# prismformore/Multi-Task-Transformer

Measured on AMD Instinct MI355X. Metric: training images/sec (512x512, 6 tasks), higher is better.
Workload: dtype f32(bf16x3)

## Files before the change

include/mtt_hip.h:

```cpp
#ifndef MTT_HIP_H
#define MTT_HIP_H

#include <stddef.h>
#include <stdint.h>

#ifdef __cplusplus
extern "C" {
#endif

#define MTT_ABI_VERSION 17

enum { MTT_F32 = 0, MTT_BF16 = 1, MTT_SPLIT = 2 };
enum { MTT_PREC_BF16 = 0, MTT_PREC_X3 = 1 };
enum { MTT_E_BADARG = -1, MTT_E_ALIGN = -2, MTT_E_UNSUPPORTED = -3 };

enum {
  MTT_OP_K = 0,
  MTT_OP_R = 1,
  MTT_OP_CONV_K = 2,
  MTT_OP_CONV_R = 3
};
enum { MTT_ACT_NONE = 0, MTT_ACT_GELU = 1, MTT_ACT_RELU = 2, MTT_ACT_GELU_BWD = 3, MTT_ACT_RELU_BWD = 4,
       MTT_ACT_GELU_DAUX = 5 ,
       MTT_ACT_MUL_AUX = 6    };
// ... 20 lines not shown
  int32_t M, N, K;
  int32_t a_op, b_op;
  int32_t a_dtype, b_dtype, d_dtype;
  int32_t prec;
  int64_t lda, ldb, ldd;
  int32_t a_mb; int64_t a_bs;
  int32_t d_mb; int64_t d_bs;
  int32_t batch, batch_inner;
  int64_t a_zo, a_zi, b_zo, b_zi, d_zo, d_zi;
  mtt_conv_geom conv;
  float alpha;
  const float* colscale; const float* colshift; int64_t col_zo, col_zi;
  int32_t act;
  const void* aux_in; void* aux_out; int32_t aux_dtype; int64_t ldaux; int64_t aux_zo, aux_zi;
  const float* rowscale; int32_t n_prompt;
  const float* resid; int64_t ldr; int32_t r_mb; int64_t r_bs; int64_t r_zo, r_zi;
  int32_t n_store;
  int32_t store_mode;
  int32_t ps_H, ps_W, ps_Co;
  int32_t variant;
  const void* A_lo; const void* B_lo; void* D_lo;
  float* colsum_out; float* colsum_ws;
  const float* a_scale; const float* a_shift; int32_t a_act; void* a_aux16; int64_t ld_a16;
} mtt_gemm_desc;
size_t mtt_gemm_colsum_ws_floats(const mtt_gemm_desc* d);

int mtt_abi_version(void);
size_t mtt_desc_size(int which);
int mtt_gemm(const mtt_gemm_desc* d, void* stream);
int mtt_gemm_variant(const mtt_gemm_desc* d);

typedef struct {
  const void* qkv; void* out; float* rawlog; float* lse;
  int32_t B, N, nH, T;
  int32_t dtype, prec;
  float scale;
  int32_t variant;
  const void* qkv_lo; void* out_lo;
} mtt_attn_desc;
int mtt_attn_fwd(const mtt_attn_desc* d, void* stream);
int mtt_attn_bwd(const mtt_attn_desc* d, const void* dout, const float* drawlog, void* dqkv, float* stat, void* stream);

typedef struct {
  const void* S; void* P; const void* dP; void* dS; const float* extra;
  int64_t rows, cols, ld; int32_t s_dtype, p_dtype; float scale;
  int64_t rows_per_mat; int32_t extra_rows; int64_t extra_ld;
} mtt_softmax_desc;
int mtt_softmax_fwd(const mtt_softmax_desc* d, void* stream);
int mtt_softmax_bwd(const mtt_softmax_desc* d, void* stream);

typedef struct {
  const float* x; void* y; const float* gamma; const float* beta; float* mean; float* rstd;
  const void* dy; float* dx; float* dgamma; float* dbeta;
// ... 317 lines not shown
```

multi-task-transformer_amd/_lib.py:

```python
import ctypes as C
import os

import torch

_HERE = os.path.dirname(os.path.abspath(__file__))
LIB_PATH = os.path.join(_HERE, "libmtt_hip.so")

ABI_VERSION = 17
F32, BF16, SPLIT = 0, 1, 2
PREC_BF16, PREC_X3 = 0, 1
OP_K, OP_R, OP_CONV_K, OP_CONV_R = 0, 1, 2, 3
ACT_NONE, ACT_GELU, ACT_RELU, ACT_GELU_BWD, ACT_RELU_BWD, ACT_GELU_DAUX, ACT_MUL_AUX = 0, 1, 2, 3, 4, 5, 6
STORE_ROWS, STORE_PIXSHUF2 = 0, 1
GEMM_AUTO, GEMM_GENERAL, GEMM_DMA256, GEMM_DMA128, GEMM_GENERAL_EPILOGUE = 0, 1, 3, 4, 11
ATTN_AUTO, ATTN_PLAIN = 0, 1

i32, i64, f32, ptr = C.c_int32, C.c_int64, C.c_float, C.c_void_p


class ConvGeom(C.Structure):
    _fields_ = [("H", i32), ("W", i32), ("C", i32), ("Cp", i32), ("dil", i32), ("flip", i32)]


class GemmDesc(C.Structure):
# ... 1 lines not shown
        ("A", ptr), ("B", ptr), ("D", ptr),
        ("M", i32), ("N", i32), ("K", i32),
        ("a_op", i32), ("b_op", i32),
        ("a_dtype", i32), ("b_dtype", i32), ("d_dtype", i32),
        ("prec", i32),
        ("lda", i64), ("ldb", i64), ("ldd", i64),
        ("a_mb", i32), ("a_bs", i64),
        ("d_mb", i32), ("d_bs", i64),
        ("batch", i32), ("batch_inner", i32),
        ("a_zo", i64), ("a_zi", i64), ("b_zo", i64), ("b_zi", i64), ("d_zo", i64), ("d_zi", i64),
        ("conv", ConvGeom),
        ("alpha", f32),
        ("colscale", ptr), ("colshift", ptr), ("col_zo", i64), ("col_zi", i64),
        ("act", i32),
        ("aux_in", ptr), ("aux_out", ptr), ("aux_dtype", i32), ("ldaux", i64), ("aux_zo", i64), ("aux_zi", i64),
        ("rowscale", ptr), ("n_prompt", i32),
        ("resid", ptr), ("ldr", i64), ("r_mb", i32), ("r_bs", i64), ("r_zo", i64), ("r_zi", i64),
        ("n_store", i32), ("store_mode", i32),
        ("ps_H", i32), ("ps_W", i32), ("ps_Co", i32),
        ("variant", i32),
        ("A_lo", ptr), ("B_lo", ptr), ("D_lo", ptr),
        ("colsum_out", ptr), ("colsum_ws", ptr),
        ("a_scale", ptr), ("a_shift", ptr), ("a_act", i32), ("a_aux16", ptr), ("ld_a16", i64),
    ]


class AttnDesc(C.Structure):
    _fields_ = [("qkv", ptr), ("out", ptr), ("rawlog", ptr), ("lse", ptr),
                ("B", i32), ("N", i32), ("nH", i32), ("T", i32), ("dtype", i32), ("prec", i32), ("scale", f32),
                ("variant", i32), ("qkv_lo", ptr), ("out_lo", ptr)]


class SoftmaxDesc(C.Structure):
    _fields_ = [("S", ptr), ("P", ptr), ("dP", ptr), ("dS", ptr), ("extra", ptr),
                ("rows", i64), ("cols", i64), ("ld", i64), ("s_dtype", i32), ("p_dtype", i32), ("scale", f32),
                ("rows_per_mat", i64), ("extra_rows", i32), ("extra_ld", i64)]


class LnDesc(C.Structure):
    _fields_ = [("x", ptr), ("y", ptr), ("gamma", ptr), ("beta", ptr), ("mean", ptr), ("rstd", ptr),
                ("dy", ptr), ("dx", ptr), ("dgamma", ptr), ("dbeta", ptr),
                ("rows", i64), ("C", i32), ("ldx", i64), ("ldy", i64), ("y_dtype", i32), ("eps", f32), ("dx_in", ptr), ("ws", ptr),
                ("y_lo", ptr), ("y32", ptr), ("ldy32", i64)]


class ChanLogitDesc(C.Structure):
# ... 335 lines not shown
    return t.data_ptr()


def _stream():
    return torch.cuda.current_stream().cuda_stream


def gemm_variant(**kw):
    lib = load()
    desc = GemmDesc()
    for k, v in kw.items():
        if k == "conv":
            for ck, cv in v.items():
                setattr(desc.conv, ck, int(cv))
        elif isinstance(v, torch.Tensor):
            setattr(desc, k, v.data_ptr())
        elif v is not None:
            setattr(desc, k, v)
    lib.mtt_gemm_variant.restype = C.c_int
    lib.mtt_gemm_variant.argtypes = [C.POINTER(GemmDesc)]
    return lib.mtt_gemm_variant(C.byref(desc))


def call(name, **kw):
    lib = load()
    fn = getattr(lib, "mtt_" + name)
    if name in POSITIONAL:
        args = [(_addr(a) if isinstance(a, torch.Tensor) else a) for a in kw["args"]]
        rc = fn(*args, _stream())
    else:
        extra = None
        if name in DESC_EXTRA:
            st, _ = DESC_EXTRA[name]
            desc = st()
            extra = [(_addr(a) if isinstance(a, torch.Tensor) else a) for a in kw["xargs"]]
        else:
            desc = (POSTPROC[name] if name in POSTPROC else EVAL[name] if name in EVAL else DESCS[name])()
        for k, v in kw.items():
            if k == "xargs":
                continue
            if k == "in":
                k = "in_"
            if k == "conv":
                for ck, cv in v.items():
                    setattr(desc.conv, ck, int(cv))
            elif isinstance(v, torch.Tensor):
# ... 13 lines not shown
```

multi-task-transformer_amd/autograd_path.py:

```python
import math

import torch
import torch.distributed as dist
import torch.nn as nn
from torch.autograd import Function

from . import bn as bn_mod
from . import _lib, ops
from ._lib import ACT_GELU, ACT_GELU_BWD, ACT_GELU_DAUX, ACT_MUL_AUX, ACT_NONE, F32, OP_CONV_R, OP_K, OP_R, dtype_code

pitch = ops.pitch
SPLITK_MIN_ROWS = 4096
WGRAD_MAX_SLICES, WGRAD_TARGET_WGS = 192, 512


def _gemm(A, B, D, M, N, K, prec, **kw):
    args = dict(A=A, B=B, D=D, M=M, N=N, K=K, a_op=OP_K, b_op=OP_K, a_dtype=dtype_code(A), b_dtype=dtype_code(B),
                d_dtype=dtype_code(D), prec=prec.code, batch=1, batch_inner=1, alpha=1.0)
    args.update(kw)
    ops.call("gemm", **args)
    return D


def _colsum(x2d, cols):
    return ops.colsum(x2d, cols)


def _scaled(g, rowscale, mb, n_prompt, prec):
    if rowscale is None and (g.dtype == prec.adt or not FAST_BWD):
        return g
    out = torch.empty(g.shape, dtype=prec.adt, device=g.device)
    ops.call("rowscale_cast", args=[g, out, g.shape[0], g.shape[1], g.stride(0), out.stride(0), dtype_code(g), dtype_code(out),
                                    rowscale, mb, n_prompt])
    return out


def _scaled_colsum(g, rowscale, mb, n_prompt, prec):
    cols = g.shape[1]
    if (rowscale is None and (g.dtype == prec.adt or not FAST_BWD)) or cols % 8 or g.stride(0) % 8:
        out = _scaled(g, rowscale, mb, n_prompt, prec)
        return out, _colsum(out, cols)
    out = torch.empty(g.shape, dtype=prec.adt, device=g.device)
    cs = torch.empty(cols, dtype=torch.float32, device=g.device)
    ws = ops.workspace(_lib.load().mtt_rowscale_cast_colsum_ws_floats(g.shape[0], cols), g.device)
    ops.call("rowscale_cast_colsum", args=[g, out, g.shape[0], cols, g.stride(0), out.stride(0), dtype_code(g), dtype_code(out),
                                           rowscale, mb, n_prompt, cs, ws])
    return out, cs


def _to_bwd(t, prec):
    if prec.name != "bf16" or t.dtype != torch.float32 or not FAST_BWD:
        return t
    t2 = t.reshape(-1, t.shape[-1])
    return ops.cast_rows(t2, torch.bfloat16).view(t.shape)


def _wgrad(dy, x, N, Kp, prec, rows=None, lda=None, ldb=None):
    rows = rows if rows is not None else dy.shape[0]
    lda, ldb = lda or dy.stride(0), ldb or x.stride(0)
    tiles = -(-N // 128) * -(-Kp // 128)
    if tiles < 96 and rows >= SPLITK_MIN_ROWS:
        Z = max(2, min(WGRAD_MAX_SLICES, WGRAD_TARGET_WGS // tiles, max(2, rows // 512)))
        c = rows // Z
        rem = rows - c * Z
        slabs = torch.empty(Z + (1 if rem else 0), N, Kp, dtype=torch.float32, device=dy.device)
        _gemm(dy, x, slabs, N, Kp, c, prec, a_op=OP_R, b_op=OP_R, lda=lda, ldb=ldb, ldd=Kp, batch=Z, a_zo=c * lda, b_zo=c * ldb,
              d_zo=N * Kp)
        if rem:
            _gemm(dy[c * Z:], x[c * Z:], slabs[Z], N, Kp, rem, prec, a_op=OP_R, b_op=OP_R, lda=lda, ldb=ldb, ldd=Kp)
        return slabs.sum(0)
# ... 220 lines not shown
        else:
            cq = ops.linear(xn, wt, hw, ps, bias=btt[None], a_rows=(T, N * C, C), M=B * T)[0]
        if side:
            xnc = xn if split or ps.adt == xn.dtype else ops.cast2d(xn, xn.shape[0], C, C, ps.adt, ldd=C)
            rawchan = ops.chan_logits(cq, xnc, B, T, N, C, (h, w), (nwin, nwin))
        pr = XT2.view(B, N, C)[:, :T]
        ops.linear(cq, wt1, C, ps, bias=btt1[None], out=pr, d_rows=(T, N * C, C), resid=pr, rowscale=rowscale, n_prompt=T, M=B * T)
    saved = (XT, g1, mean, rstd, ops._hi(xn), ops._hi(qkv), ops._hi(ao), ops._hi(wq), ops._hi(wp), rowscale, lse, cq, wt, wt1, xp32) if keep else None
    return (XT2, rawlog, rawchan), saved


def mlp_half(XT2, g2, b2n, eps, W1, b1, W2, b2, rowscale, geo, prec, tag, *, keep, pe=None):
    B, N, T = geo
    pe = pe or prec
    assert not keep or pe.name == prec.name
    C, Hd = W1.shape[1], W1.shape[0]
    split = prec.split and ((C % 64 == 0 and Hd % 64 == 0) if MLP_SPLIT_RULE64 else (ops.split_gemm_ok(C) and ops.split_gemm_ok(Hd)))
    odt = "split" if split else prec.adt
    xn2, mean, rstd = ops.layernorm(XT2, g2, b2n, eps, prec, save_stats=keep, out_dtype=odt)
    w1 = ops.pack_linear([W1], pe, tag + ('fc1',), split=split)
    w2 = ops.pack_linear([W2], pe, tag + ('fc2',), split=split)
    z = torch.empty(B * N, Hd, dtype=prec.bwd.adt, device=XT2.device) if keep else None
    daux = keep and GELU_DAUX and z.dtype == torch.bfloat16
    hmid = ops.linear(xn2, w1, Hd, pe, bias=b1[None], act=ACT_GELU_DAUX if daux else ACT_GELU, aux_out=z, out_dtype=odt)[0]
    XT3 = torch.empty_like(XT2)
    rows = dict(d_rows=(N, N * C, C), M=B * N) if keep or rowscale is not None else {}
    ops.linear(hmid, w2, C, pe, bias=b2[None], out=XT3, resid=XT2, rowscale=rowscale, n_prompt=T, **rows)
    saved = (XT2, g2, mean, rstd, ops._hi(xn2), z, ops._hi(hmid), ops._hi(w1), ops._hi(w2), rowscale) if keep else None
    return XT3, saved


class AttnHalfFn(Function):

    @staticmethod
    def forward(ctx, XT, g1, b1, eps, Wqkv, bqkv, Wproj, bproj, Wtt, btt, Wtt1, btt1, rowscale, geo, prec, tag):
        (XT2, rawlog, rawchan), saved = attn_half(XT, g1, b1, eps, Wqkv, bqkv, Wproj, bproj, Wtt, btt, Wtt1, btt1, rowscale, geo, prec, tag, keep=True)
        ctx.save_for_backward(*saved)
        ctx.geo, ctx.prec, ctx.eps, ctx.chan = geo, prec, eps, Wtt is not None
        ctx.params = (Wqkv, Wproj, Wtt, Wtt1)
        ctx.set_materialize_grads(False)
        z = torch.zeros(0, device=XT.device)
        return XT2, (rawlog if rawlog is not None else z), (rawchan if rawchan is not None else z)

    @staticmethod
    def backward(ctx, dXT2, drawlog, drawchan):
        XT, g1, mean, rstd, xn, qkv, ao, wq, wp, rowscale, lse, cq, wt, wt1, xp32 = ctx.saved_tensors
        Wqkv_, Wproj_, Wtt_, Wtt1_ = ctx.params
        B, N, nH, T, h, w, nwin = ctx.geo[:7]
        prec, C, M, hw = ctx.prec.bwd, nH * 64, B * N, h * w
        xn_c = xn
        if dXT2 is None:
            dXT2 = torch.zeros_like(XT)
        dXT2 = dXT2.contiguous()
        g, dbproj = _scaled_colsum(dXT2, rowscale, N, T, prec)
        dWproj, _ = _enc_wgrad(g, ao, C, C, prec, bias=False)
        dao = _enc_dgrad(g, Wproj_, wp[0], M, C, C, prec, prec.adt, 'proj')
        dl = drawlog.contiguous() if (T > 0 and drawlog is not None and drawlog.numel()) else None
        if lse is not None:
            dqkv = attention_bwd_flash(qkv, ao, lse, dao, dl, B, N, nH, T, prec)
        else:
            dqkv = attention_bwd(qkv, dao, dl, B, N, nH, T, prec)
        dWqkv, dbqkv = _enc_wgrad(dqkv, xn, 3 * C, C, prec)
        dxn = _enc_dgrad(dqkv, Wqkv_, wq[0], M, C, 3 * C, prec, torch.float32, 'qkv')
        dWtt = dbtt = dWtt1 = dbtt1 = None
        if ctx.chan:
            hwp = cq.shape[-1]
            gp = dXT2.view(B, N, C)[:, :T].reshape(B * T, C)
            if rowscale is not None:
                gp = gp * rowscale[:, 0].repeat_interleave(T)[:, None]
            dWtt1 = _wgrad(gp, cq, C, hwp, prec)[:, :hw]
            dbtt1 = _colsum(gp, C)
            fast_tt = prec.name == "bf16" and FAST_BWD and hwp == hw and hw >= FAST_MIN_DIM and C >= FAST_MIN_DIM and C % 64 == 0
            if fast_tt:
                gp16 = ops.cast_rows(gp, torch.bfloat16)
                dcq = _enc_dgrad(gp16, Wtt1_, wt1[0], B * T, hwp, C, prec, torch.float32, 'tt1')
            else:
                dcq = _dgrad(gp, wt1[0], B * T, hwp, C, prec, torch.float32)
            if drawchan is not None and drawchan.numel():
                dq2 = torch.zeros(B * T, hwp, dtype=torch.float32, device=xn.device)
# ... 18 lines not shown


class MlpHalfFn(Function):

    @staticmethod
    def forward(ctx, XT2, g2, b2n, eps, W1, b1, W2, b2, rowscale, geo, prec, tag):
        XT3, saved = mlp_half(XT2, g2, b2n, eps, W1, b1, W2, b2, rowscale, geo, prec, tag, keep=True)
        ctx.save_for_backward(*saved)
        ctx.geo, ctx.prec, ctx.eps, ctx.daux = geo, prec, eps, GELU_DAUX and saved[5].dtype == torch.bfloat16
        ctx.params = (W1, W2)
        return XT3

    @staticmethod
    def backward(ctx, dXT3):
        XT2, g2, mean, rstd, xn2, z, hmid, w1, w2, rowscale = ctx.saved_tensors
        B, N, T = ctx.geo
        prec, M = ctx.prec.bwd, B * N
        C, Hd = xn2.shape[1], z.shape[1]
        dXT3 = dXT3.contiguous()
        g, db2 = _scaled_colsum(dXT3, rowscale, N, T, prec)
        W1_, W2_ = ctx.params
        dW2, _ = _enc_wgrad(g, hmid, C, Hd, prec, bias=False)
        dz, db1 = _enc_dgrad(g, W2_, w2[0], M, Hd, C, prec, prec.adt, 'fc2', colsum=True, act=ACT_MUL_AUX if ctx.daux else ACT_GELU_BWD, aux_in=z,
                             aux_dtype=dtype_code(z), ldaux=Hd)
        dW1, _ = _enc_wgrad(dz, xn2, Hd, C, prec, bias=False)
        dxn2 = _enc_dgrad(dz, W1_, w1[0], M, C, Hd, prec, prec.adt, 'fc1')
        dXT2, dg2, dbn2 = _ln_bwd_join(dXT3, XT2, dxn2, g2, mean, rstd, ctx.eps)
        return dXT2, dg2, dbn2, None, dW1, db1, dW2, db2, None, None, None, None


def block_attn(keep, gp, *args):
    return AttnHalfFn.apply(*args) if keep else attn_half(*args, keep=False, gp=gp)[0]


def block_mlp(keep, pe, *args):
    return MlpHalfFn.apply(*args) if keep else mlp_half(*args, keep=False, pe=pe)[0]


def patch_embed(img, Wpe, bpe, pos, first, geo, prec, tag, pe=None):
    B, N, T, hw = geo
    C = Wpe.shape[0]
    XT = torch.empty(B * N, C, dtype=torch.float32, device=img.device)
    XT.view(B, N, C)[:, :T] = first
    cols = ops.patchify(img.float(), prec)
    wpe = ops.pack_linear([Wpe], pe or prec, tag)
    ops.linear(cols, wpe, C, pe or prec, bias=bpe[None], out=XT.view(B, N, C)[:, T:], d_rows=(hw, N * C, C),
               resid=pos[0, 1:], r_rows=(hw, 0, C), M=B * hw)
    return XT, cols

# ... 700 lines not shown
```

multi-task-transformer_amd/csrc/gemm.hip:

```cpp
#include "mtt_device.h"
#include <type_traits>

namespace {

#ifndef MTT_GROUP_M
#define MTT_GROUP_M 4
#endif
#ifndef MTT_RING
#define MTT_RING 1
#endif
constexpr int BM = 128, BN = 128, BK = 64;
constexpr int TILE_BYTES = BM * BK * 2;

struct GemmP {
  mtt_gemm_desc d;
  FastDiv divW, divH, divCp, div3;
  FastDiv divAmb, divDmb, divRmb;
  FastDiv divPsW, divPsH, divPsCo;
  int tiles_m, tiles_n;
  int group_m;
#ifdef MTT_GEMM_TRACE
  unsigned long long* trace;
#endif
};

#ifdef MTT_GEMM_TRACE
MTT_DEV unsigned long long trace_hwid() {
  unsigned a, b;
  asm volatile("s_getreg_b32 %0, hwreg(HW_REG_HW_ID)" : "=s"(a));
  asm volatile("s_getreg_b32 %0, hwreg(HW_REG_XCC_ID)" : "=s"(b));
  return (unsigned long long)a | ((unsigned long long)b << 32);
}
#define MTT_TRACE(slot) do { if (p.trace && threadIdx.x == 0) p.trace[(size_t)(blockIdx.x + gridDim.x * blockIdx.z) * 8 + (slot)] = __builtin_amdgcn_s_memtime(); } while (0)
#define MTT_TRACE_RT(slot) do { if (p.trace && threadIdx.x == 0) p.trace[(size_t)(blockIdx.x + gridDim.x * blockIdx.z) * 8 + (slot)] = __builtin_amdgcn_s_memrealtime(); } while (0)
#define MTT_TRACE_ID(tile) do { if (p.trace && threadIdx.x == 0) { p.trace[(size_t)(blockIdx.x + gridDim.x * blockIdx.z) * 8 + 6] = trace_hwid(); p.trace[(size_t)(blockIdx.x + gridDim.x * blockIdx.z) * 8 + 7] = (tile); } } while (0)
#else
#define MTT_TRACE(slot) do {} while (0)
#define MTT_TRACE_RT(slot) do {} while (0)
#define MTT_TRACE_ID(tile) do {} while (0)
#endif

MTT_DEV int64_t row_off(uint32_t m, int mb, int64_t bs, int64_t ld, FastDiv f) {
  if (mb <= 0) return (int64_t)m * ld;
  const uint32_t q = fdiv(m, f);
  return (int64_t)q * bs + (int64_t)(m - q * (uint32_t)mb) * ld;
}


__device__ __attribute__((aligned(32))) const unsigned g_zero_page[8] = {0u, 0u, 0u, 0u, 0u, 0u, 0u, 0u};

template <bool X3, bool CONV, bool F32>
struct StagerK {
  const void* base; int dtype; int K; int c;
  int64_t roff[4]; bool rok[4];
  uint64_t zpage;
  unsigned tapmask[4];
  int tap, ci, knext;
  Raw8<F32> raw[4];

  MTT_DEV void init(const GemmP& p, const void* b, int dt, int row0, int rows, int64_t ld, int mb, int64_t bs, FastDiv fmb) {
    base = b; dtype = dt; K = p.d.K; c = threadIdx.x & 7;
    zpage = (uint64_t)(uintptr_t)g_zero_page;
    asm volatile("" : "+s"(zpage));
#pragma unroll
    for (int i = 0; i < 4; ++i) {
      const int r = row0 + (threadIdx.x >> 3) + 32 * i;
      rok[i] = r < rows;
      const uint32_t rr = rok[i] ? (uint32_t)r : 0u;
// ... 699 lines not shown
    } else {
      const int k0 = s * BK;
#pragma unroll
      for (int i = 0; i < 4; ++i) {
        const uint64_t src = (uint64_t)(uintptr_t)(Abase + (aoff[i] + k0));
        glds16((const bf16_t*)(uintptr_t)(k0 + ack[i] < K ? src : zpage), sA + i * 1024);
      }
#pragma unroll
      for (int i = 0; i < 4; ++i) {
        const uint64_t src = (uint64_t)(uintptr_t)(Bbase + (boff[i] + k0));
        glds16((const bf16_t*)(uintptr_t)(k0 + ack[i] < K ? src : zpage), sB + i * 1024);
      }
    }
  };

  f32x4 acc[MT][NT];
#pragma unroll
  for (int a = 0; a < MT; ++a)
#pragma unroll
    for (int b = 0; b < NT; ++b) acc[a][b] = (f32x4){0.f, 0.f, 0.f, 0.f};

  const int nk = X3CAT ? 3 * (K / BK) : (K + BK - 1) / BK;
  issue(0, 0);
  asm volatile("s_waitcnt vmcnt(0)" ::: "memory");
  __builtin_amdgcn_s_barrier();
  MTT_TRACE(2);
  if (late) __builtin_amdgcn_s_barrier();
  __builtin_amdgcn_sched_barrier(0);

  auto main_loop = [&](auto late_tag) {
  (void)late_tag;
  for (int kt = 0; kt < nk; ++kt) {
    const unsigned char* Ah = smem + (kt & 1) * STAGE;
    const unsigned char* Bh = Ah + TILE_A;
#pragma unroll
    for (int kh = 0; kh < 2; ++kh) {
      if (kh == 0 && kt + 1 < nk) issue((kt + 1) & 1, kt + 1);
      u32x4 fa[MT], fb[NT];
#pragma unroll
      for (int t = 0; t < NT; ++t) fb[t] = *(const u32x4*)(Bh + lds_off(wn * 64 + t * 16 + li, kh * 4 + lg));
#pragma unroll
      for (int t = 0; t < MT; ++t) fa[t] = *(const u32x4*)(Ah + lds_off(wm * (MT * 16) + t * 16 + li, kh * 4 + lg));
      if (kh == 1) asm volatile("s_waitcnt vmcnt(0) lgkmcnt(0)" ::: "memory");
      else asm volatile("s_waitcnt lgkmcnt(0)" ::: "memory");
      __builtin_amdgcn_sched_barrier(0);
      __builtin_amdgcn_s_barrier();
      __builtin_amdgcn_sched_barrier(0);
      __builtin_amdgcn_s_setprio(1);
#pragma unroll
      for (int a = 0; a < MT; ++a)
#pragma unroll
        for (int b = 0; b < NT; ++b) acc[a][b] = mfma16(fa[a], fb[b], acc[a][b]);
      __builtin_amdgcn_s_setprio(0);
      __builtin_amdgcn_sched_barrier(0);
      __builtin_amdgcn_s_barrier();
      __builtin_amdgcn_sched_barrier(0);
    }
  }
  };
  if (late) main_loop(std::true_type{}); else main_loop(std::false_type{});
  if (!late) __builtin_amdgcn_s_barrier();
  __syncthreads();
  MTT_TRACE(3);
  gemm_epilogue_auto<256, WAVES_M, WAVES_N, MT, NT>(p, acc, smem, m0, n0, zo, zi);
  MTT_TRACE(4); MTT_TRACE_RT(5); MTT_TRACE_ID(tile_m * tiles_n + tile_n);
}

template <int ADDR>
int launch_dma(const GemmP& p, hipStream_t stream) {
  constexpr int smem = (BM2 * BK * 2 + 256 * BK * 2) * 2;
  static std::atomic<unsigned long long> done{0};
  if (int e = mtt_ensure_dyn_lds((const void*)gemm_dma_kernel<ADDR>, smem, done)) return e;
  const int tm = (p.d.M + BM2 - 1) / BM2, tn = (p.d.N + 255) / 256;
  dim3 grid(tm * tn, 1, p.d.batch);
  hipLaunchKernelGGL((gemm_dma_kernel<ADDR>), grid, dim3(512), smem, stream, p);
  return (int)hipGetLastError();
}

MTT_DEV int ring_swz(int row) { return (0x78 >> (((row >> 2) & 3) * 2)) & 3; }

#define MTT_VMCNT_CASE(n) case n: asm volatile("s_waitcnt vmcnt(" #n ")" ::: "memory"); break;
MTT_DEV void wait_vmcnt_dyn(int n) {
  switch (n) {
    MTT_VMCNT_CASE(24) MTT_VMCNT_CASE(22) MTT_VMCNT_CASE(20) MTT_VMCNT_CASE(18) MTT_VMCNT_CASE(16) MTT_VMCNT_CASE(14) MTT_VMCNT_CASE(12)
// ... 70 lines not shown
#pragma unroll
      for (int i = 0; i < 2; ++i) {
        const uint64_t src = (uint64_t)(uintptr_t)(base + aoff32[i]);
        glds16((const bf16_t*)(uintptr_t)(((tapmask[i] >> tap) & 1u) ? src : zpage), dst + i * 1024);
      }
      return;
    }
    const unsigned char* base = (part == 0 ? AbaseH : part == 1 ? BbaseH : part == 2 ? BbaseL : AbaseL) + (size_t)j * 64;
    glds16((const bf16_t*)(base + (isA ? aoff32[0] : boff32[0])), dst);
    if (isA || !EDGE) glds16((const bf16_t*)(base + (isA ? aoff32[1] : boff32[1])), dst + 1024);
  };
  const int fsw = ((lg ^ ring_swz(li)) << 4) + li * 64;
  const int fragA = wm * (MT * 16) * 64 + fsw, fragB = wn * (NT * 16) * 64 + fsw;

  f32x4 acc[MT][NT];
#pragma unroll
  for (int a = 0; a < MT; ++a)
#pragma unroll
    for (int b = 0; b < NT; ++b) acc[a][b] = (f32x4){0.f, 0.f, 0.f, 0.f};

  constexpr int W_BL = 3 * NA + 2 * NB, W_AL = 3 * NA + 3 * NB, W_AB = 2 * NA + 3 * NB;
  issue_part(0, 0); issue_part(0, 1); issue_part(0, 2); issue_part(0, 3);
  issue_part(1, 0); issue_part(1, 1); issue_part(1, 2);
  wait_vmcnt_imm<2 * NA + 3 * NB>();
  __builtin_amdgcn_s_barrier();
  if (late) __builtin_amdgcn_s_barrier();
  __builtin_amdgcn_sched_barrier(0);

#define MTT_R3_CLOSE() do { __builtin_amdgcn_sched_barrier(0); __builtin_amdgcn_s_barrier(); __builtin_amdgcn_sched_barrier(0); } while (0)
  auto main_loop = [&](auto late_tag) {
  constexpr bool LATE = decltype(late_tag)::value;
  for (int j = 0; j < nk; ++j) {
    const unsigned char* sb = smem + (j & 1) * SLOT;
    const bool m1 = j + 1 < nk, m2 = j + 2 < nk;
    const int w_bl = NA + (m1 ? 2 * NA + 2 * NB : 0), w_al = (m1 ? 2 * NA + 2 * NB : 0) + (m2 ? NA + NB : 0), w_ab = NA + NB + (m2 ? NA + 2 * NB : 0);
    u32x4 fa[MT], fbh[NT], fbl[NT];
    if (m1) issue_part(j + 1, 3);
#pragma unroll
    for (int t = 0; t < NT; ++t) fbh[t] = *(const u32x4*)(sb + PART + fragB + t * 1024);
#pragma unroll
    for (int t = 0; t < MT; ++t) fa[t] = *(const u32x4*)(sb + fragA + t * 1024);
    if (LATE) { if (m2) wait_vmcnt_imm<W_BL>(); else wait_vmcnt_dyn(w_bl); }
    asm volatile("s_waitcnt lgkmcnt(0)" ::: "memory");
    MTT_R3_CLOSE();
    __builtin_amdgcn_s_setprio(1);
#pragma unroll
// ... 16 lines not shown
      for (int b = 0; b < NT; ++b) acc[a][b] = mfma16(fa[a], fbl[b], acc[a][b]);
    __builtin_amdgcn_s_setprio(0);
    if (!LATE) { if (m2) wait_vmcnt_imm<W_AL>(); else wait_vmcnt_dyn(w_al); }
    MTT_R3_CLOSE();
    if (m2) issue_part(j + 2, 2);
#pragma unroll
    for (int t = 0; t < MT; ++t) fa[t] = *(const u32x4*)(sb + 3 * PART + fragA + t * 1024);
    if (LATE) { if (m2) wait_vmcnt_imm<W_AB>(); else wait_vmcnt_dyn(w_ab); }
    asm volatile("s_waitcnt lgkmcnt(0)" ::: "memory");
    MTT_R3_CLOSE();
    __builtin_amdgcn_s_setprio(1);
#pragma unroll
    for (int a = 0; a < MT; ++a)
#pragma unroll
      for (int b = 0; b < NT; ++b) acc[a][b] = mfma16(fa[a], fbh[b], acc[a][b]);
    __builtin_amdgcn_s_setprio(0);
    if (!LATE) { if (m2) wait_vmcnt_imm<W_AB>(); else wait_vmcnt_dyn(w_ab); }
    MTT_R3_CLOSE();
  }
  };
#undef MTT_R3_CLOSE
  if (late) main_loop(std::true_type{}); else main_loop(std::false_type{});
  if (!late) __builtin_amdgcn_s_barrier();
  __syncthreads();
  if constexpr (EDGE) gemm_epilogue<128, WAVES_M, WAVES_N, MT, NT>(p, acc, smem, m0, n0, zo, zi);
  else gemm_epilogue_auto<256, WAVES_M, WAVES_N, MT, NT>(p, acc, smem, m0, n0, zo, zi);
}

template <bool CONV>
__global__ __launch_bounds__(512, 1) void gemm_ring3_kernel(const GemmP p) {
  extern __shared__ __attribute__((aligned(16))) unsigned char smem[];
  const int wg = xcd_remap(blockIdx.x, gridDim.x);
  const int tiles_n = (p.d.N + 255) / 256, tiles_m = (p.d.M + BM2 - 1) / BM2;
  int tile_m, tile_n;
  grouped_tile(wg, tiles_m, tiles_n, p.group_m, tile_m, tile_n);
  const int m0 = tile_m * BM2, n0 = tile_n * 256;
  const int z = blockIdx.z;
  const int zo = z / p.d.batch_inner, zi = z - zo * p.d.batch_inner;
  const int ncols = (p.d.n_store > p.d.N ? p.d.n_store : p.d.N) - n0;
  if (MTT_R3_EDGE && ncols <= 128 && p.d.store_mode == MTT_STORE_ROWS) ring3_tile<CONV, true>(p, smem, m0, n0, zo, zi);
  else ring3_tile<CONV, false>(p, smem, m0, n0, zo, zi);
}

template <bool CONV>
int launch_ring3(const GemmP& p, hipStream_t stream) {
  constexpr int smem = 2 * 4 * 16384;
// ... 629 lines not shown
    if (fills && 100 * (int64_t)d.M * d.N >= 45 * pm * pn) return 6;
    return 0;
  }
  const bool dma = d.a_op == MTT_OP_K && d.b_op == MTT_OP_K && (d.K % 8) == 0;
  if (!dma || d.variant == MTT_GEMM_GENERAL) return 0;
  if (d.variant == MTT_GEMM_DMA256) return 3;
  if (d.variant == MTT_GEMM_DMA128) return 4;
  const int n256 = (d.N + 255) / 256 * 256, n128 = (d.N + 127) / 128 * 128;
  const bool wide = 100 * n128 > 85 * n256;
  const int batch = d.batch < 1 ? 1 : d.batch;
  const int64_t blocks = (int64_t)((d.M + 255) / 256) * ((d.N + 255) / 256) * batch;
  if (wide && d.M >= 512 && d.N >= 512 && blocks >= 96) return 3;
  const int tbn = 32 * dma128_nt(d);
  const int64_t blocks128 = (int64_t)((d.M + 127) / 128) * ((d.N + tbn - 1) / tbn) * batch;
  if (d.M >= 512 && d.K >= 128 && blocks128 >= 256) return 4;
  if (d.M >= 128 && d.N >= 256 && d.K >= 512) return 4;
  return 0;
}
#ifdef MTT_GEMM_TRACE
static unsigned long long* g_trace_host = nullptr;
extern "C" void mtt_debug_set_trace(void* buf) { g_trace_host = (unsigned long long*)buf; }
#endif
extern "C" int mtt_gemm_variant(const mtt_gemm_desc* d) { return d ? gemm_variant_for(*d) : MTT_E_BADARG; }

static int gemm_launch(GemmP& p, hipStream_t s, int v);
extern "C" int mtt_gemm(const mtt_gemm_desc* dd, void* stream) {
  if (!dd || !dd->A || !dd->B || !dd->D) return MTT_E_BADARG;
  GemmP p; p.d = *dd;
  mtt_gemm_desc& d = p.d;
  if (d.M <= 0 || d.N <= 0 || d.K <= 0) return MTT_E_BADARG;
  if (d.batch < 1) d.batch = 1;
  if (d.batch_inner < 1) d.batch_inner = 1;
  const bool a_k = d.a_op == MTT_OP_K || d.a_op == MTT_OP_CONV_K, b_k = d.b_op == MTT_OP_K;
  const int Kp8 = (d.K + 7) / 8 * 8;
  if ((a_k && d.a_op == MTT_OP_K && d.lda < Kp8) || (b_k && d.ldb < Kp8)) return MTT_E_ALIGN;
  if (d.a_op == MTT_OP_CONV_K && (d.K % 8)) return MTT_E_ALIGN;
  if ((d.lda % 8) || (d.ldb % 8)) return MTT_E_ALIGN;
  if (((uintptr_t)d.A & 15) || ((uintptr_t)d.B & 15)) return MTT_E_ALIGN;
  if ((d.aux_in || d.aux_out) && (d.ldaux <= 0 || (d.ldaux % 8))) return MTT_E_BADARG;
  if (d.act < MTT_ACT_NONE || d.act > MTT_ACT_MUL_AUX) return MTT_E_BADARG;
  if ((d.act == MTT_ACT_GELU_DAUX && !d.aux_out) || ((d.act == MTT_ACT_MUL_AUX || d.act == MTT_ACT_GELU_BWD || d.act == MTT_ACT_RELU_BWD) && !d.aux_in))
    return MTT_E_BADARG;
  if ((d.ldd % 8) || ((uintptr_t)d.D & 15) || (d.d_bs % 8) || (d.d_zo % 8) || (d.d_zi % 8)) return MTT_E_ALIGN;
  if (d.resid && ((d.ldr % 4) || ((uintptr_t)d.resid & 15) || (d.r_bs % 4))) return MTT_E_ALIGN;
  const bool conv = d.a_op == MTT_OP_CONV_K || d.b_op == MTT_OP_CONV_R;
  if (conv) {
    if (d.conv.H <= 0 || d.conv.W <= 0 || d.conv.Cp % 8 || d.conv.C > d.conv.Cp || d.conv.dil < 1) return MTT_E_BADARG;
    if (d.a_op == MTT_OP_CONV_K && d.K != 9 * d.conv.Cp) return MTT_E_BADARG;
    if (d.b_op == MTT_OP_CONV_R && d.N != 9 * d.conv.Cp) return MTT_E_BADARG;
  }
  if (d.store_mode == MTT_STORE_PIXSHUF2 && (d.ps_H <= 0 || d.ps_W <= 0 || d.ps_Co <= 0 || d.N != 4 * d.ps_Co)) return MTT_E_BADARG;
  p.divW = make_div(conv ? d.conv.W : 1); p.divH = make_div(conv ? d.conv.H : 1);
  p.divCp = make_div(conv ? d.conv.Cp : 1); p.div3 = make_div(3);
  p.divAmb = make_div(d.a_mb > 0 ? d.a_mb : 1); p.divDmb = make_div(d.d_mb > 0 ? d.d_mb : 1);
  p.divRmb = make_div(d.r_mb > 0 ? d.r_mb : 1);
  p.divPsW = make_div(d.ps_W > 0 ? d.ps_W : 1); p.divPsH = make_div(d.ps_H > 0 ? d.ps_H : 1);
  p.divPsCo = make_div(d.ps_Co > 0 ? d.ps_Co : 1);
  p.tiles_m = (d.M + BM - 1) / BM; p.tiles_n = (d.N + BN - 1) / BN;
  p.group_m = MTT_GROUP_M;
#ifdef MTT_GEMM_TRACE
  p.trace = g_trace_host;
#endif
  hipStream_t s = (hipStream_t)stream;
  const int v = gemm_variant_for(d);
  if (v < 0) return v;
  if (d.d_dtype == MTT_SPLIT && !d.D_lo) return MTT_E_BADARG;
  if (d.d_dtype == MTT_SPLIT && d.store_mode != MTT_STORE_ROWS) return MTT_E_UNSUPPORTED;
  if (d.colsum_out) {
    if (!d.colsum_ws) return MTT_E_BADARG;
    if (d.batch != 1 || d.store_mode != MTT_STORE_ROWS || v == 6) return MTT_E_UNSUPPORTED;
    const int rc = gemm_launch(p, s, v);
    if (rc) return rc;
    const int tbm = (v == 3 || v == 8 || v == 9) ? 256 : BM;
    hipLaunchKernelGGL(mtt_colsum_final_kernel, dim3((d.N + 31) / 32, 1, 1), dim3(256), 0, s, (const float*)d.colsum_ws, d.colsum_out, d.N,
                       (d.M + tbm - 1) / tbm, (int64_t)0);
    return (int)hipGetLastError();
  }
  return gemm_launch(p, s, v);
}

// ... 46 lines not shown
```

multi-task-transformer_amd/ops.py:

```python
import weakref

import torch

from . import _lib
from ._lib import (ACT_GELU, ACT_NONE, ACT_RELU, BF16, F32, OP_CONV_K, OP_CONV_R, OP_K, OP_R, PREC_BF16, PREC_X3, SPLIT)


PITCH32_FROM = 160


def pitch(n):
    return (n + 31) // 32 * 32 if n >= PITCH32_FROM else (n + 7) // 8 * 8


DEFAULT_PREC = "x3f"


class Prec:

    def __init__(self, name):
        assert name in ("bf16", "x3", "x3f")
        self.name = name
        self.code = PREC_BF16 if name == "bf16" else PREC_X3
        self.adt = torch.bfloat16 if name == "bf16" else torch.float32
# ... 371 lines not shown
    mode, dt = _mode(prec, split)
    return seg_pack((tag, mode, 'kmap', tuple(id(w) for w in weights)), list(weights),
                    lambda: _dest((Z, N, Kp), dt, weights[0].device),
                    lambda buf: [segment(w, s0, buf, z * N * Kp + d0, (1, N, ln), (0, K, 1), (0, Kp, 1))
                                 for z, w in enumerate(weights) for (d0, s0, ln) in kmap],
                    check=lambda: _check_sources(weights, lambda w: w.numel() == N * K))


def stack_vec(vs, tag):
    n, Z = vs[0].numel(), len(vs)
    if any(v.dtype != torch.float32 or not v.is_contiguous() or v.numel() != n for v in vs):
        def build():
            with torch.no_grad():
                return torch.stack([v.detach().float().reshape(-1) for v in vs], 0).contiguous()
        return _cached((tag, tuple(id(v) for v in vs)), vs, build)
    return seg_pack((tag, 'vec', tuple(id(v) for v in vs)), list(vs),
                    lambda: torch.zeros(Z, n, dtype=torch.float32, device=vs[0].device),
                    lambda buf: [segment(v, 0, buf, z * n, (1, 1, n), (0, 0, 1), (0, 0, 1)) for z, v in enumerate(vs)])



def linear(x, wpack, N, prec, *, bias=None, act=ACT_NONE, out=None, out_dtype=None, M=None,
           a_rows=None, d_rows=None, resid=None, r_rows=None, rowscale=None, n_prompt=0, aux_out=None, aux_in=None,
           colscale=None, alpha=1.0, batch_inner=1, d_z=None, ldd=None, n_store=None, a_affine=None):
    Z, Nw, Kp = wpack.shape
    assert N <= Nw
    x_split = isinstance(x, Split)
    assert x_split == isinstance(wpack, Split), "split planes: both operands or neither"
    if a_rows is not None:
        a_mb, a_bs, lda = a_rows
        a_z = 0
    else:
        xh = _hi(x)
        xv = xh if xh.dim() == 3 else xh[None]
        if M is None:
            M = xv.shape[1]
        a_mb, a_bs, lda = 0, 0, xv.shape[2]
        a_z = xv.stride(0) if xv.shape[0] > 1 else 0
        assert xv.shape[0] in (1, Z) and lda >= Kp
    Np = ldd if (out is None and ldd is not None) else pitch(N)
    if out is None:
        out = Split.empty((Z, M, Np), x.device) if out_dtype == "split" else torch.empty(Z, M, Np, dtype=out_dtype or prec.adt, device=x.device)
    oh = _hi(out)
    if d_rows is not None:
        d_mb, d_bs, ldd_ = d_rows
        dz = 0
        nst = N
# ... 13 lines not shown
        kw.update(A_lo=x.lo, B_lo=wpack.lo)
    if isinstance(out, Split):
        kw.update(D_lo=out.lo)
    kw.update(a_zo=a_z * batch_inner, a_zi=a_z if batch_inner > 1 else 0,
              b_zo=wh.stride(0) * batch_inner, b_zi=wh.stride(0) if batch_inner > 1 else 0)
    if d_z is not None:
        kw.update(d_zo=d_z[0], d_zi=d_z[1])
    else:
        kw.update(d_zo=dz * batch_inner, d_zi=dz if batch_inner > 1 else 0)
    if bias is not None or colscale is not None:
        ref = bias if bias is not None else colscale
        cz = ref.stride(0) if (ref.dim() == 2 and ref.shape[0] > 1) else 0
        kw.update(colshift=bias, colscale=colscale, col_zo=cz * batch_inner, col_zi=cz if batch_inner > 1 else 0)
    if resid is not None:
        rr = r_rows if r_rows is not None else (d_mb, d_bs, ldd_)
        kw.update(resid=resid, r_mb=rr[0], r_bs=rr[1], ldr=rr[2])
    if rowscale is not None:
        kw.update(rowscale=rowscale, n_prompt=n_prompt)
    if aux_out is not None or aux_in is not None:
        aux = aux_out if aux_out is not None else aux_in
        az = aux.stride(0) if aux.dim() == 3 else 0
        kw.update(aux_out=aux_out, aux_in=aux_in, aux_dtype=dtype_code(aux), ldaux=aux.shape[-1],
                  aux_zo=az * batch_inner, aux_zi=az if batch_inner > 1 else 0)
    if a_affine is not None:
        sc, sh, a_act, a16 = a_affine
        kw.update(a_scale=sc, a_shift=sh, a_act=a_act, a_aux16=a16, ld_a16=a16.stride(-2) if a16 is not None else 0)
    call("gemm", **kw)
    return out


def head_prologue_ok(rows, K, n, lda):
    return GEMM_VARIANT is None and n <= 32 and K % 8 == 0 and K <= 1024 and rows >= 1 and lda % 4 == 0


SPLIT_CONV_MAX_ELEMS = 2 ** 31 - 1


def conv3x3(x, wpack, Co, Ci, B, H, W, prec, *, bias=None, colscale=None, act=ACT_NONE, dil=1, flip=0, out_dtype=None):
    Z, rows, Cp = x.shape
    assert rows == B * H * W and wpack.shape[-1] == 9 * Cp
    if isinstance(wpack, Split) and not isinstance(x, Split):
        x = x.float().contiguous()
        sp = split_cast(x.view(Z * rows, Cp))
        x = Split(sp.hi.view(Z, rows, Cp), sp.lo.view(Z, rows, Cp))
    assert isinstance(x, Split) == isinstance(wpack, Split), "split planes: both operands or neither"
    Cop = pitch(Co)
# ... 262 lines not shown
```

Before: 189.0.

## Skip GEMM main loop for row tiles fully zeroed by drop-path rowscale

Adds a per-tile check in two GEMM kernel paths that reads the per-sample rowscale table. When every row in a 128-row tile belongs to a sample whose drop-path scale is zero, the K-loop is skipped and only the epilogue runs on a zero accumulator. Encoder MLP fc1 forward and the proj, fc2 and fc1 dgrad calls pass this table as a hint, so samples dropped by stochastic depth stop costing matrix math. The cost is a small per-tile table read, plus reliance on downstream rowscale masking to zero out the bias/activation values that are still written for skipped rows. A runtime toggle is exposed for debugging.

```diff
diff --git a/include/mtt_hip.h b/include/mtt_hip.h
--- a/include/mtt_hip.h
+++ b/include/mtt_hip.h
@@ -66,6 +66,7 @@
   const void* A_lo; const void* B_lo; void* D_lo;
   float* colsum_out; float* colsum_ws;
   const float* a_scale; const float* a_shift; int32_t a_act; void* a_aux16; int64_t ld_a16;
+  const float* skip_scale; int32_t skip_mb, skip_np;
 } mtt_gemm_desc;
 size_t mtt_gemm_colsum_ws_floats(const mtt_gemm_desc* d);
 
@@ -73,6 +74,7 @@
 size_t mtt_desc_size(int which);
 int mtt_gemm(const mtt_gemm_desc* d, void* stream);
 int mtt_gemm_variant(const mtt_gemm_desc* d);
+int mtt_debug_set_gemm_rowskip(int on);
 
 typedef struct {
   const void* qkv; void* out; float* rawlog; float* lse;
diff --git a/multi-task-transformer_amd/_lib.py b/multi-task-transformer_amd/_lib.py
--- a/multi-task-transformer_amd/_lib.py
+++ b/multi-task-transformer_amd/_lib.py
@@ -47,6 +47,7 @@
         ("A_lo", ptr), ("B_lo", ptr), ("D_lo", ptr),
         ("colsum_out", ptr), ("colsum_ws", ptr),
         ("a_scale", ptr), ("a_shift", ptr), ("a_act", i32), ("a_aux16", ptr), ("ld_a16", i64),
+        ("skip_scale", ptr), ("skip_mb", i32), ("skip_np", i32),
     ]
 
 
@@ -428,6 +429,13 @@
     return lib.mtt_gemm_variant(C.byref(desc))
 
 
+def set_gemm_rowskip(on):
+    lib = load()
+    lib.mtt_debug_set_gemm_rowskip.restype = C.c_int
+    lib.mtt_debug_set_gemm_rowskip.argtypes = [C.c_int]
+    return bool(lib.mtt_debug_set_gemm_rowskip(1 if on else 0))
+
+
 def call(name, **kw):
     lib = load()
     fn = getattr(lib, "mtt_" + name)
diff --git a/multi-task-transformer_amd/autograd_path.py b/multi-task-transformer_amd/autograd_path.py
--- a/multi-task-transformer_amd/autograd_path.py
+++ b/multi-task-transformer_amd/autograd_path.py
@@ -46,6 +46,12 @@
     ops.call("rowscale_cast_colsum", args=[g, out, g.shape[0], cols, g.stride(0), out.stride(0), dtype_code(g), dtype_code(out),
                                            rowscale, mb, n_prompt, cs, ws])
     return out, cs
+
+
+def _skip_hint(rowscale, mb, n_prompt):
+    if rowscale is None or not rowscale.is_cuda:
+        return {}
+    return dict(skip_scale=rowscale, skip_mb=mb, skip_np=n_prompt)
 
 
 def _to_bwd(t, prec):
@@ -312,7 +318,8 @@
     w2 = ops.pack_linear([W2], pe, tag + ('fc2',), split=split)
     z = torch.empty(B * N, Hd, dtype=prec.bwd.adt, device=XT2.device) if keep else None
     daux = keep and GELU_DAUX and z.dtype == torch.bfloat16
-    hmid = ops.linear(xn2, w1, Hd, pe, bias=b1[None], act=ACT_GELU_DAUX if daux else ACT_GELU, aux_out=z, out_dtype=odt)[0]
+    hmid = ops.linear(xn2, w1, Hd, pe, bias=b1[None], act=ACT_GELU_DAUX if daux else ACT_GELU, aux_out=z, out_dtype=odt,
+                      row_skip=_skip_hint(rowscale, N, T))[0]
     XT3 = torch.empty_like(XT2)
     rows = dict(d_rows=(N, N * C, C), M=B * N) if keep or rowscale is not None else {}
     ops.linear(hmid, w2, C, pe, bias=b2[None], out=XT3, resid=XT2, rowscale=rowscale, n_prompt=T, **rows)
@@ -344,7 +351,7 @@
         dXT2 = dXT2.contiguous()
         g, dbproj = _scaled_colsum(dXT2, rowscale, N, T, prec)
         dWproj, _ = _enc_wgrad(g, ao, C, C, prec, bias=False)
-        dao = _enc_dgrad(g, Wproj_, wp[0], M, C, C, prec, prec.adt, 'proj')
+        dao = _enc_dgrad(g, Wproj_, wp[0], M, C, C, prec, prec.adt, 'proj', **_skip_hint(rowscale, N, T))
         dl = drawlog.contiguous() if (T > 0 and drawlog is not None and drawlog.numel()) else None
         if lse is not None:
             dqkv = attention_bwd_flash(qkv, ao, lse, dao, dl, B, N, nH, T, prec)
@@ -409,9 +416,9 @@
         W1_, W2_ = ctx.params
         dW2, _ = _enc_wgrad(g, hmid, C, Hd, prec, bias=False)
         dz, db1 = _enc_dgrad(g, W2_, w2[0], M, Hd, C, prec, prec.adt, 'fc2', colsum=True, act=ACT_MUL_AUX if ctx.daux else ACT_GELU_BWD, aux_in=z,
-                             aux_dtype=dtype_code(z), ldaux=Hd)
+                             aux_dtype=dtype_code(z), ldaux=Hd, **_skip_hint(rowscale, N, T))
         dW1, _ = _enc_wgrad(dz, xn2, Hd, C, prec, bias=False)
-        dxn2 = _enc_dgrad(dz, W1_, w1[0], M, C, Hd, prec, prec.adt, 'fc1')
+        dxn2 = _enc_dgrad(dz, W1_, w1[0], M, C, Hd, prec, prec.adt, 'fc1', **_skip_hint(rowscale, N, T))
         dXT2, dg2, dbn2 = _ln_bwd_join(dXT3, XT2, dxn2, g2, mean, rstd, ctx.eps)
         return dXT2, dg2, dbn2, None, dW1, db1, dW2, db2, None, None, None, None
 
diff --git a/multi-task-transformer_amd/csrc/gemm.hip b/multi-task-transformer_amd/csrc/gemm.hip
--- a/multi-task-transformer_amd/csrc/gemm.hip
+++ b/multi-task-transformer_amd/csrc/gemm.hip
@@ -9,6 +9,9 @@
 #ifndef MTT_RING
 #define MTT_RING 1
 #endif
+#ifndef MTT_GEMM_ROWSKIP
+#define MTT_GEMM_ROWSKIP 1
+#endif
 constexpr int BM = 128, BN = 128, BK = 64;
 constexpr int TILE_BYTES = BM * BK * 2;
 
@@ -17,6 +20,9 @@
   FastDiv divW, divH, divCp, div3;
   FastDiv divAmb, divDmb, divRmb;
   FastDiv divPsW, divPsH, divPsCo;
+  const float* skip_tab;
+  int skip_mb, skip_np;
+  FastDiv divSkip;
   int tiles_m, tiles_n;
   int group_m;
 #ifdef MTT_GEMM_TRACE
@@ -44,6 +50,20 @@
   if (mb <= 0) return (int64_t)m * ld;
   const uint32_t q = fdiv(m, f);
   return (int64_t)q * bs + (int64_t)(m - q * (uint32_t)mb) * ld;
+}
+
+MTT_DEV bool rows_all_dropped(const GemmP& p, int m0, int m1) {
+  if (!MTT_GEMM_ROWSKIP || !p.skip_tab) return false;
+  uint32_t q = fdiv((uint32_t)m0, p.divSkip);
+  int r0 = m0 - (int)q * p.skip_mb;
+  for (int m = m0; m < m1; ++q) {
+    const int left = m1 - m, room = p.skip_mb - r0;
+    const int n = left < room ? left : room;
+    if (r0 < p.skip_np && p.skip_tab[2 * q] != 0.0f) return false;
+    if (r0 + n > p.skip_np && p.skip_tab[2 * q + 1] != 0.0f) return false;
+    m += n; r0 = 0;
+  }
+  return true;
 }
 
 
@@ -789,8 +809,10 @@
 
   const int nk = X3CAT ? 3 * (K / BK) : (K + BK - 1) / BK;
   issue(0, 0);
+  const bool dropped = ADDR == 1 && rows_all_dropped(p, m0, m0 + BM2 < p.d.M ? m0 + BM2 : p.d.M);
   asm volatile("s_waitcnt vmcnt(0)" ::: "memory");
   __builtin_amdgcn_s_barrier();
+  if (!dropped) {
   MTT_TRACE(2);
   if (late) __builtin_amdgcn_s_barrier();
   __builtin_amdgcn_sched_barrier(0);
@@ -827,6 +849,7 @@
   };
   if (late) main_loop(std::true_type{}); else main_loop(std::false_type{});
   if (!late) __builtin_amdgcn_s_barrier();
+  }
   __syncthreads();
   MTT_TRACE(3);
   gemm_epilogue_auto<256, WAVES_M, WAVES_N, MT, NT>(p, acc, smem, m0, n0, zo, zi);
@@ -943,6 +966,9 @@
   constexpr int W_BL = 3 * NA + 2 * NB, W_AL = 3 * NA + 3 * NB, W_AB = 2 * NA + 3 * NB;
   issue_part(0, 0); issue_part(0, 1); issue_part(0, 2); issue_part(0, 3);
   issue_part(1, 0); issue_part(1, 1); issue_part(1, 2);
+  const bool dropped = !CONV && rows_all_dropped(p, m0, m0 + BM2 < p.d.M ? m0 + BM2 : p.d.M);
+  if (dropped) asm volatile("s_waitcnt vmcnt(0)" ::: "memory");
+  else {
   wait_vmcnt_imm<2 * NA + 3 * NB>();
   __builtin_amdgcn_s_barrier();
   if (late) __builtin_amdgcn_s_barrier();
@@ -1005,6 +1031,7 @@
 #undef MTT_R3_CLOSE
   if (late) main_loop(std::true_type{}); else main_loop(std::false_type{});
   if (!late) __builtin_amdgcn_s_barrier();
+  }
   __syncthreads();
   if constexpr (EDGE) gemm_epilogue<128, WAVES_M, WAVES_N, MT, NT>(p, acc, smem, m0, n0, zo, zi);
   else gemm_epilogue_auto<256, WAVES_M, WAVES_N, MT, NT>(p, acc, smem, m0, n0, zo, zi);
@@ -1680,6 +1707,8 @@
 extern "C" void mtt_debug_set_trace(void* buf) { g_trace_host = (unsigned long long*)buf; }
 #endif
 extern "C" int mtt_gemm_variant(const mtt_gemm_desc* d) { return d ? gemm_variant_for(*d) : MTT_E_BADARG; }
+static std::atomic<int> g_rowskip_on{1};
+extern "C" int mtt_debug_set_gemm_rowskip(int on) { return g_rowskip_on.exchange(on ? 1 : 0); }
 
 static int gemm_launch(GemmP& p, hipStream_t s, int v);
 extern "C" int mtt_gemm(const mtt_gemm_desc* dd, void* stream) {
@@ -1714,6 +1743,13 @@
   p.divRmb = make_div(d.r_mb > 0 ? d.r_mb : 1);
   p.divPsW = make_div(d.ps_W > 0 ? d.ps_W : 1); p.divPsH = make_div(d.ps_H > 0 ? d.ps_H : 1);
   p.divPsCo = make_div(d.ps_Co > 0 ? d.ps_Co : 1);
+  if (d.skip_scale && (d.skip_mb <= 0 || d.skip_np < 0)) return MTT_E_BADARG;
+  p.skip_tab = nullptr; p.skip_mb = 1; p.skip_np = 0;
+  if (g_rowskip_on.load(std::memory_order_relaxed)) {
+    if (d.rowscale && d.d_mb > 0) { p.skip_tab = d.rowscale; p.skip_mb = d.d_mb; p.skip_np = d.n_prompt; }
+    else if (!d.rowscale && d.skip_scale) { p.skip_tab = d.skip_scale; p.skip_mb = d.skip_mb; p.skip_np = d.skip_np; }
+  }
+  p.divSkip = make_div(p.skip_mb);
   p.tiles_m = (d.M + BM - 1) / BM; p.tiles_n = (d.N + BN - 1) / BN;
   p.group_m = MTT_GROUP_M;
 #ifdef MTT_GEMM_TRACE
diff --git a/multi-task-transformer_amd/ops.py b/multi-task-transformer_amd/ops.py
--- a/multi-task-transformer_amd/ops.py
+++ b/multi-task-transformer_amd/ops.py
@@ -417,7 +417,7 @@
 
 def linear(x, wpack, N, prec, *, bias=None, act=ACT_NONE, out=None, out_dtype=None, M=None,
            a_rows=None, d_rows=None, resid=None, r_rows=None, rowscale=None, n_prompt=0, aux_out=None, aux_in=None,
-           colscale=None, alpha=1.0, batch_inner=1, d_z=None, ldd=None, n_store=None, a_affine=None):
+           colscale=None, alpha=1.0, batch_inner=1, d_z=None, ldd=None, n_store=None, a_affine=None, row_skip=None):
     Z, Nw, Kp = wpack.shape
     assert N <= Nw
     x_split = isinstance(x, Split)
@@ -477,6 +477,8 @@
         az = aux.stride(0) if aux.dim() == 3 else 0
         kw.update(aux_out=aux_out, aux_in=aux_in, aux_dtype=dtype_code(aux), ldaux=aux.shape[-1],
                   aux_zo=az * batch_inner, aux_zi=az if batch_inner > 1 else 0)
+    if row_skip:
+        kw.update(row_skip)
     if a_affine is not None:
         sc, sh, a_act, a16 = a_affine
         kw.update(a_scale=sc, a_shift=sh, a_act=a_act, a_aux16=a16, ld_a16=a16.stride(-2) if a16 is not None else 0)
```

Result: no change. 189.0, median of 2 (+0.0%).
